# jwh97nn/AnyRef

Hardware: AMD Instinct MI355X
Metric: images/sec (1024^2, 7B LLM+ViT-L+SAM-H) (higher is better)
Workload: dtype bf16 (LLaMA / CLIP) + f16 (SAM encoder)

## Files before the change

### anyref_amd/_lib.py

```python
from __future__ import annotations

import ctypes as C
import os

import torch

HERE = os.path.dirname(os.path.abspath(__file__))
LIB_PATH = os.path.join(HERE, "libanyref_hip.so")

ABI_VERSION = 2
F32, BF16, F16 = 0, 1, 2
MODE_PARITY, MODE_PERF, MODE_PERF_FP8W, MODE_PARITY16 = 0, 1, 2, 3


class AnyrefConfig(C.Structure):
    _fields_ = [
        ("abi_version", C.c_int32), ("mode", C.c_int32),
        ("clip_image", C.c_int32), ("clip_patch", C.c_int32), ("clip_dim", C.c_int32),
        ("clip_heads", C.c_int32), ("clip_layers_run", C.c_int32), ("clip_mlp", C.c_int32),
        ("clip_eps", C.c_float),
        ("llm_vocab", C.c_int32), ("llm_dim", C.c_int32), ("llm_heads", C.c_int32),
        ("llm_layers", C.c_int32), ("llm_mlp", C.c_int32), ("llm_max_seq", C.c_int32),
        ("llm_rms_eps", C.c_float), ("llm_rope_theta", C.c_float),
        ("sam_img", C.c_int32), ("sam_patch", C.c_int32), ("sam_dim", C.c_int32), ("sam_depth", C.c_int32),
        ("sam_heads", C.c_int32), ("sam_mlp_ratio", C.c_int32), ("sam_window", C.c_int32),
        ("sam_n_global", C.c_int32), ("sam_global_idx", C.c_int32 * 8),
        ("sam_out_chans", C.c_int32), ("dec_heads", C.c_int32), ("dec_mlp", C.c_int32),
        ("dec_depth", C.c_int32), ("num_mask_tokens", C.c_int32),
        ("out_dim", C.c_int32), ("audio_dim", C.c_int32),
        ("seg_lo", C.c_int32), ("seg_hi", C.c_int32),
        ("rephrase_weight", C.c_float),
        ("max_batch", C.c_int32), ("max_seg", C.c_int32),
        ("aud_dim", C.c_int32), ("aud_blocks", C.c_int32), ("aud_heads", C.c_int32), ("aud_mel", C.c_int32),
        ("aud_len", C.c_int32), ("aud_kernel", C.c_int32), ("aud_stride", C.c_int32), ("aud_clips", C.c_int32),
    ]


_P = C.c_void_p
_I = C.c_int
_F = C.c_float
_L = C.c_int64

SYMBOLS = {
    "anyref_create": (_I, [C.POINTER(AnyrefConfig), _I, C.POINTER(_P)]),
    "anyref_destroy": (None, [_P]),
    "anyref_last_error": (C.c_char_p, [_P]),
    "anyref_set_weight": (_I, [_P, C.c_char_p, _P, _I, _I, C.POINTER(_L), _I]),
    "anyref_finalize": (_I, [_P]),
    "anyref_generate": (_I, [_P, _P, _P, _P, _P, _P, _I, _I, _P, _P, _I, _P, _P, _I, _I, _P, _P, _P, _P, _L, _P,
                             _P, _P]),
    "anyref_forward_teacher": (_I, [_P, _P, _P, _P, _P, _P, _I, _I, _P, _P, _I, _P, _P, _P, _P, _P, _L, _P, _P,
                                    _P, _P]),
    "anyref_encode_images": (_I, [_P, _P, _P, _I, _P, _P]),
    "anyref_sam_encode": (_I, [_P, _P, _P, _I, _P]),
    "anyref_mask_decode": (_I, [_P, _P, _P, _P, _I, _P, _P, _P, _P, _P]),
    "anyref_llm_forward": (_I, [_P, _P, _P, _P, _I, _I, _P, _P, _P, _P]),
    "anyref_project_audio": (_I, [_P, _P, _P, _I, _P]),
    "anyref_audio_encode": (_I, [_P, _P, _P, _I, _P]),
    "anyref_seg_tail": (_I, [_P, _P, _P, _P, _P, _P, _I, _I, _I, _P, _I, _P, _P, _P, _P, _P, _L, _P, _P]),
    "anyref_set_seg_range": (_I, [_P, _I, _I]),
    "anyref_set_overlap": (_I, [_P, _I]),
    "anyref_set_early_tail": (_I, [_P, _I]),
    "anyref_set_extra_event": (_I, [_P, _P]),
    "anyref_set_graphs": (_I, [_P, _I]),
    "anyref_set_side_share": (_I, [_P, _I, _I]),
    "anyref_profile_enable": (_I, [_P, _I]),
    "anyref_profile_config": (_I, [_P, C.c_char_p, _I]),
    "anyref_profile_collect": (_I, [_P]),
    "anyref_profile_calibrate": (_I, [_P, _P, C.POINTER(C.c_double)]),
    "anyref_profile_read": (_I, [_P, _I, C.c_char_p, _I, C.POINTER(C.c_double), C.POINTER(_L),
                                C.POINTER(C.c_double), C.POINTER(C.c_double)]),
    "anyref_stamps_enable": (_I, [_P, _I]),
    "anyref_stamps_collect": (_I, [_P, C.POINTER(_L)]),
    "anyref_stamps_dropped": (_I, [_P, C.POINTER(_L)]),
    "anyref_stamps_read": (_I, [_P, _L, C.c_char_p, _I, C.POINTER(C.c_double), C.POINTER(C.c_double),
                               C.POINTER(C.c_double), C.POINTER(_I)]),
    "anyref_stamps_spread": (_I, [_P, _L, C.POINTER(C.c_double), C.POINTER(C.c_double), C.POINTER(C.c_double)]),
    "anyref_device_bytes": (_L, [_P]),
    "anyref_mode_name": (C.c_char_p, [_P]),
    "anyref_op_gemm": (_I, [_I, _P, _P, _P, _P, _P, _P, _P, _I, _I, _I, _I, _I]),
    "anyref_op_gemm_fp8": (_I, [_P, _P, _P, _P, _P, _P, _P, _I, _I, _I, _I, _I]),
    "anyref_op_quant_fp8": (_I, [_P, _P, _I, _I, _P, _P]),
    "anyref_op_gemv_fp8": (_I, [_P, _P, _P, _F, _P, _P, _P, _P, _P, _P, _I, _I, _I]),
    "anyref_op_iou_counts": (_I, [_P, _P, _P, _I, _L, _P]),
    "anyref_op_avs_counts": (_I, [_P, _P, _P, _I, _L, _P, _I, _F, _P, _P]),
    "anyref_op_sam_preprocess": (_I, [_P, _P, _I, _I, _I, C.POINTER(C.c_float), C.POINTER(C.c_float), _P]),
    "anyref_op_pil_resample_u8": (_I, [_P, _P, _I, _I, _I, _P, _P, _I, _I, _P, _P, _I, _P, _P, _I]),
    "anyref_op_pool_ref_tokens": (_I, [_P, _P, _I, _I, _I, _I, _P]),
    "anyref_op_kaldi_fbank": (_I, [_P, _P, _I, _I, _I, _I, _I, C.c_float, _P, _I, _P, _P, _I, C.c_float, C.c_float, _P]),
    "anyref_op_clip_finish": (_I, [_P, _P, _I, _I, _I, _I, _I, _I, _I, C.POINTER(C.c_float), C.POINTER(C.c_float), _P]),
    "anyref_op_gemv": (_I, [_I, _P, _P, _P, _F, _P, _P, _P, _P, _P, _I, _I, _I, _I]),
    "anyref_op_norm": (_I, [_I, _P, _P, _P, _P, _P, _I, _I, _F, _I]),
    "anyref_op_attention": (_I, [_I, _P, _P, _P, _P, _P, _I, _I, _I, _I, _I, _F, _I, _P, _P, _P, _I, _I]),
    "anyref_op_attention_tab": (_I, [_I, _P, _P, _P, _P, _P, _I, _I, _I, _I, _F, _P, _P, _I, _I, _I]),
    "anyref_op_gemm_gather": (_I, [_I, _P, _P, _P, _P, _P, _P, _P, _I, _I, _I, _I]),
    "anyref_op_attention_relp": (_I, [_I, _P, _P, _P, _P, _P, _I, _I, _I, _I, _F, _P, _I, _I, _I]),
    "anyref_op_rel_pos": (_I, [_I, _P, _P, _P, _P, _I, _I, _I, _I, _P, _P]),
    "anyref_op_postprocess": (_I, [_P, _P, _I, _I, _I, _I, _I, _I, _I, _I, _P]),
    "anyref_op_last_error": (C.c_char_p, []),
}

_lib = None


def load() -> C.CDLL:
    global _lib
    if _lib is not None:
        return _lib
    if not os.path.exists(LIB_PATH):
        raise RuntimeError(
            f"{LIB_PATH} not found: build the HIP backend first "
            "(`python -c 'import __graft_entry__ as g; g.build()'` or `make -C anyref_amd/csrc`). "
            "anyref_amd has no CPU fallback.")
    lib = C.CDLL(LIB_PATH)
    for name, (res, args) in SYMBOLS.items():
        fn = getattr(lib, name)
        fn.restype = res
        fn.argtypes = args
    _lib = lib
    return lib
```

### anyref_amd/csrc/gemm_impl.h

```cpp
#include <algorithm>
#include <cmath>
#include <cstdlib>
#include <stdexcept>
#include <type_traits>
#include <utility>
#include <vector>
#include <mutex>

#pragma once
#include "kernels.h"

namespace anyref {

template <typename T>
struct Mma;
template <>
struct Mma<bf16> {
  static constexpr int KS = 32;
  static constexpr int VEC = 8;
  using Frag = short8;
  static __device__ inline Frag load(const bf16* p, int lane) {
    return *reinterpret_cast<const short8*>(p + 8 * (lane >> 4));
  }
  static __device__ inline float4v mma(Frag a, Frag b, float4v c) {
// ... 280 lines not shown
                  ? *reinterpret_cast<const uint4v*>(A + (int64_t)gm * a.lda + gk)
                  : uint4v{0, 0, 0, 0};
    }
#pragma unroll
    for (int i = 0; i < WV; ++i) {
      const int v = tid + i * 256, row = v / KV, kv = v % KV;
      const int gn = n0 + row, gk = k0 + kv * VEC;
      rw[i] = (gn < a.N && gk < a.K)
                  ? *reinterpret_cast<const uint4v*>(W + (int64_t)gn * a.ldw + gk)
                  : uint4v{0, 0, 0, 0};
    }
  };
  auto sstore = [&]() {
#pragma unroll
    for (int i = 0; i < AV; ++i) {
      const int v = tid + i * 256, row = v / KV, kv = v % KV;
      *reinterpret_cast<uint4v*>(&As[row * LD + kv * VEC]) = ra[i];
    }
#pragma unroll
    for (int i = 0; i < WV; ++i) {
      const int v = tid + i * 256, row = v / KV, kv = v % KV;
      *reinterpret_cast<uint4v*>(&Ws[row * LD + kv * VEC]) = rw[i];
    }
  };

  gload(0);
  for (int k0 = 0; k0 < a.K; k0 += BK) {
    sstore();
    __syncthreads();
    if (k0 + BK < a.K) gload(k0 + BK);
#pragma unroll
    for (int ks = 0; ks < BK / KS; ++ks) {
      typename M_::Frag af[MI], bf[NI];
#pragma unroll
      for (int i = 0; i < MI; ++i)
        af[i] = M_::load(&As[(wr * (BM / 2) + i * 16 + (lane & 15)) * LD + ks * KS], lane);
#pragma unroll
      for (int j = 0; j < NI; ++j)
        bf[j] = M_::load(&Ws[(wc * (BN / 2) + j * 16 + (lane & 15)) * LD + ks * KS], lane);
#pragma unroll
      for (int i = 0; i < MI; ++i)
#pragma unroll
        for (int j = 0; j < NI; ++j) acc[i][j] = M_::mma(bf[j], af[i], acc[i][j]);
    }
    __syncthreads();
  }

  gemm_epilogue<T, MI, NI>(a, acc, m0 + wr * (BM / 2), n0 + wc * (BN / 2), z, lane);
}

typedef const __attribute__((address_space(1))) void* gas_ptr;
typedef __attribute__((address_space(3))) void* las_ptr;

template <int N>
__device__ __forceinline__ void wait_vmcnt() {
  asm volatile("s_waitcnt vmcnt(%0)" ::"n"(N) : "memory");
}

__device__ __forceinline__ short8 fp8x8_to_bf16x8(uint2v r) {
  short8 o;
#pragma unroll
  for (int h = 0; h < 2; ++h) {
    const float2v lo = __builtin_amdgcn_cvt_pk_f32_fp8((int)r[h], false);
    const float2v hi = __builtin_amdgcn_cvt_pk_f32_fp8((int)r[h], true);
    o[4 * h] = (short)f2bf(lo[0]).x; o[4 * h + 1] = (short)f2bf(lo[1]).x;
    o[4 * h + 2] = (short)f2bf(hi[0]).x; o[4 * h + 3] = (short)f2bf(hi[1]).x;
  }
  return o;
}

template <int BM, int BN, int WM, int WN, int NS, bool W8 = false, bool PERSIST = false, typename TT = bf16>
__global__ __launch_bounds__(WM * WN * 64) void gemm_glds_kernel(GemmArgs a) {
  using T = TT;
  constexpr bool SPLIT = is_split<TT>::value;
  using ET = std::conditional_t<SPLIT, bf16, TT>;
  constexpr int AX = SPLIT ? 2 : 1;
  static_assert(!W8 || !(is_half16<T>::value || SPLIT), "fp8 weights are widened to bf16");
  constexpr int BK = 64, NW = WM * WN;
  constexpr int TM = BM / WM, TN = BN / WN, MI = TM / 16, NI = TN / 16;
  constexpr int ROWB = BK * 2;
  constexpr int WROWB = W8 ? BK : BK * 2;
  constexpr int WRPI = W8 ? 16 : 8;
  constexpr int TILEB = BM * ROWB + BN * WROWB;
  constexpr int RA = BM / (NW * 8), RWF = BN / (NW * WRPI), PW = (BN % (NW * WRPI)) / WRPI, RW = RWF + (PW > 0);
  constexpr int LPT = RA + RWF;
#ifdef ANYREF_GEMM_NO_PAIRW
  constexpr bool PAIRW = false;
#else
  constexpr bool PAIRW = !W8 && !(NI % 2 == 1 && BM < 256);
#endif
  constexpr int NIP = PAIRW ? (NI & ~1) : 0;
  static_assert(BM % (NW * 8) == 0 && BN % WRPI == 0 && (PW == 0 || !W8), "tile rows must split over the waves");
  static_assert(NS >= 2 && NS <= 4 && (NS - 2) * (LPT + 1) <= 63, "stage count / vmcnt range");
  extern __shared__ __attribute__((aligned(1024))) char smem[];
  const int tid = threadIdx.x, lane = tid & 63, wave = __builtin_amdgcn_readfirstlane(tid >> 6);
  const int wr = wave / WN, wc = wave % WN;
  auto wswz = [](int row) { return PAIRW ? ((row >> 1) & 1) | (((row >> 3) & 3) << 1) : (row >> 1) & 7; };
  auto wrow = [&](int f) {
    const int i = lane & 15;
    return wc * TN + (f < NIP ? (f >> 1) * 32 + 8 * (i >> 2) + 4 * (f & 1) + (i & 3) : f * 16 + i);
  };
  const int tiles_m = cdiv(a.M, BM), tiles_n = cdiv(a.N, BN), nwg = tiles_m * tiles_n;
  for (int vb = blockIdx.x; vb < nwg; vb += gridDim.x) {
  int id = vb;
  if (a.order & 1) {
    const int q = nwg / 8, r = nwg % 8, xcd = id % 8;
    id = (xcd < r ? xcd * (q + 1) : r * (q + 1) + (xcd - r) * q) + id / 8;
  }
  int tm, tn;
  if (a.group_m > 0) {
    const int per = a.group_m * tiles_n, g = id / per, first = g * a.group_m;
    const int gsz = tiles_m - first < a.group_m ? tiles_m - first : a.group_m;
    tm = first + (id % per) % gsz;
    tn = (id % per) / gsz;
  } else {
    tm = (a.order & 2) ? id % tiles_m : id / tiles_n;
    tn = (a.order & 2) ? id / tiles_m : id % tiles_n;
  }
  const int m0 = tm * BM, n0 = tn * BN;
  const int z = blockIdx.z;
  const ET* __restrict__ A = reinterpret_cast<const ET*>(a.A) + (int64_t)z * a.sA * AX;
  using WT = std::conditional_t<W8, uint8_t, ET>;
  const WT* __restrict__ W = reinterpret_cast<const WT*>(a.W) + (int64_t)z * a.sW;

  float4v acc[MI][NI];
#pragma unroll
  for (int i = 0; i < MI; ++i)
#pragma unroll
    for (int j = 0; j < NI; ++j) acc[i][j] = float4v{0.f, 0.f, 0.f, 0.f};

  const int srow = lane >> 3, sp = lane & 7;
  const ET* asrc[RA];
  const WT* wsrc[RW];
#pragma unroll
  for (int r = 0; r < RA; ++r) {
    const int row = (r * NW + wave) * 8 + srow;
    int gm = m0 + row;
    gm = gm < a.M ? gm : a.M - 1;
    if (a.a_row_map) gm = a.a_row_map[gm];
    asrc[r] = A + (int64_t)gm * a.lda * AX + ((sp ^ ((row >> 1) & 7)) << 3);
  }
#pragma unroll
  for (int r = 0; r < RW; ++r) {
    if constexpr (W8) {
      const int row = (r * NW + wave) * 16 + (lane >> 2);
      int gn = n0 + row;
      gn = gn < a.N ? gn : a.N - 1;
      wsrc[r] = W + (int64_t)gn * a.ldw + (((lane & 3) ^ ((row >> 2) & 3)) << 4);
    } else {
      const int row = (r * NW + wave) * 8 + srow;
      int gn = n0 + row;
      gn = gn < a.N ? gn : a.N - 1;
      wsrc[r] = W + (int64_t)gn * a.ldw + ((sp ^ wswz(row)) << 3);
    }
  }
  auto stage = [&](auto buf_c, int t) {
    constexpr int buf = decltype(buf_c)::value;
    char* base = smem + buf * TILEB;
#pragma unroll
    for (int r = 0; r < RA; ++r)
      __builtin_amdgcn_global_load_lds((gas_ptr)(asrc[r] + t * BK), (las_ptr)(base + (r * NW + wave) * 8 * ROWB), 16, 0,
                                       0);
#pragma unroll
    for (int r = 0; r < RW; ++r)
      if (r < RWF || wave < PW)
        __builtin_amdgcn_global_load_lds((gas_ptr)(wsrc[r] + (SPLIT ? t >> 1 : t) * BK),
                                         (las_ptr)(base + BM * ROWB + (r * NW + wave) * WRPI * WROWB), 16, 0, 0);
  };
  auto wait_tiles = [&](auto n_c) {
    constexpr int N = decltype(n_c)::value;
    if constexpr (PW == 0 || N == 0) {
      wait_vmcnt<N * LPT>();
    } else {
      if (wave < PW) wait_vmcnt<N * (LPT + 1)>();
      else wait_vmcnt<N * LPT>();
    }
  };
  constexpr bool QUAD = BM == 256 && WM == 2 && !W8 && MI == 8 && NI == 4;
  auto compute_quad = [&](auto buf_c) {
    constexpr int buf = decltype(buf_c)::value;
    constexpr int MH = MI / 2, NH0 = NI / 2, NH1 = NI - NH0;
    const char* Ab = smem + buf * TILEB;
    const char* Wb = Ab + BM * ROWB;
    short8 a0[2][MH], a1[2][MH], b0[2][NH0], b1[2][NH1];
    auto lda = [&](auto i_c, short8 (&af)[2][MH]) {
#pragma unroll
      for (int ks = 0; ks < 2; ++ks)
#pragma unroll
        for (int f = 0; f < MH; ++f) {
          const int row = wr * TM + (decltype(i_c)::value * MH + f) * 16 + (lane & 15), c = ks * 4 + (lane >> 4);
          af[ks][f] = *reinterpret_cast<const short8*>(Ab + row * ROWB + ((c ^ ((row >> 1) & 7)) << 4));
        }
    };
    auto ldw0 = [&]() {
#pragma unroll
      for (int ks = 0; ks < 2; ++ks)
#pragma unroll
        for (int f = 0; f < NH0; ++f) {
          const int row = wrow(f), c = ks * 4 + (lane >> 4);
          b0[ks][f] = *reinterpret_cast<const short8*>(Wb + row * ROWB + ((c ^ wswz(row)) << 4));
        }
    };
    auto ldw1 = [&]() {
#pragma unroll
      for (int ks = 0; ks < 2; ++ks)
#pragma unroll
        for (int f = 0; f < NH1; ++f) {
          const int row = wrow(NH0 + f), c = ks * 4 + (lane >> 4);
          b1[ks][f] = *reinterpret_cast<const short8*>(Wb + row * ROWB + ((c ^ wswz(row)) << 4));
        }
    };
    auto mma = [&](auto i_c, auto j_c, const short8 (&af)[2][MH], const auto& bf) {
      constexpr int i = decltype(i_c)::value, j = decltype(j_c)::value, NH = j == 0 ? NH0 : NH1;
      __builtin_amdgcn_s_setprio(1);
#pragma unroll
      for (int ks = 0; ks < 2; ++ks)
#pragma unroll
        for (int f = 0; f < MH; ++f)
#pragma unroll
          for (int h = 0; h < NH; ++h)
            acc[i * MH + f][j * NH0 + h] =
                mfma_16x16x32<ET>(bf[ks][h], af[ks][f], acc[i * MH + f][j * NH0 + h]);
      __builtin_amdgcn_s_setprio(0);
    };
    using I0 = std::integral_constant<int, 0>;
    using I1 = std::integral_constant<int, 1>;
    ldw0();
    lda(I0(), a0);
    ldw1();
    mma(I0(), I0(), a0, b0);
    lda(I1(), a1);
    mma(I0(), I1(), a0, b1);
    mma(I1(), I1(), a1, b1);
    mma(I1(), I0(), a1, b0);
  };
  auto compute = [&](auto buf_c) {
    if constexpr (QUAD) {
      compute_quad(buf_c);
      return;
    }
    constexpr int buf = decltype(buf_c)::value;
    const char* Ab = smem + buf * TILEB;
    const char* Wb = Ab + BM * ROWB;
#pragma unroll
    for (int ks = 0; ks < BK / 32; ++ks) {
      short8 af[MI], bfr[NI];
      const int c = ks * 4 + (lane >> 4);
#pragma unroll
      for (int i = 0; i < MI; ++i) {
        const int row = wr * TM + i * 16 + (lane & 15);
        af[i] = *reinterpret_cast<const short8*>(Ab + row * ROWB + ((c ^ ((row >> 1) & 7)) << 4));
      }
#pragma unroll
      for (int j = 0; j < NI; ++j) {
        const int row = wrow(j);
        if constexpr (W8) {
          const int g = lane >> 4, c8 = ks * 2 + (g >> 1);
// ... 86 lines not shown
      float4v acc;
      if constexpr (SP > 0) {
        float4v t[SP];
#pragma unroll
        for (int z = 0; z < SP; ++z) t[z] = *reinterpret_cast<const float4v*>(slabs + z * slab_stride + e);
        acc = t[0];
#pragma unroll
        for (int z = 1; z < SP; ++z) acc += t[z];
      } else {
        acc = *reinterpret_cast<const float4v*>(slabs + e);
        for (int z = 1; z < splits; ++z) acc += *reinterpret_cast<const float4v*>(slabs + z * slab_stride + e);
      }
      acc *= a.alpha;
      if (a.col_scale) acc *= *reinterpret_cast<const float4v*>(a.col_scale + n);
      if (a.bias) acc += *reinterpret_cast<const float4v*>(a.bias + n);
      acc = float4v{apply_act(acc[0], a.act), apply_act(acc[1], a.act), apply_act(acc[2], a.act), apply_act(acc[3], a.act)};
      if (a.resid) acc += *reinterpret_cast<const float4v*>(a.resid + (int64_t)m * a.ldr + n);
      if (a.c_f32) {
        *reinterpret_cast<float4v*>(Cf + (int64_t)m * a.ldc + n) = acc;
      } else if constexpr (is_split<T>::value) {
        st4<T>(Ct + (int64_t)m * a.ldc, n, acc[0], acc[1], acc[2], acc[3]);
      } else {
        T* o = Ct + (int64_t)m * a.ldc + n;
        o[0] = from_f32<T>(acc[0]); o[1] = from_f32<T>(acc[1]); o[2] = from_f32<T>(acc[2]); o[3] = from_f32<T>(acc[3]);
      }
      v[i] = acc;
      ss += acc[0] * acc[0] + acc[1] * acc[1] + acc[2] * acc[2] + acc[3] * acc[3];
    } else {
      v[i] = float4v{0.f, 0.f, 0.f, 0.f};
    }
  }
  __shared__ float red[NT / 64];
  float mean = 0.f;
  if (a.norm_bias) {
    float s1 = 0.f;
#pragma unroll
    for (int i = 0; i < MAXV; ++i) s1 += v[i][0] + v[i][1] + v[i][2] + v[i][3];
    s1 = wave_sum(s1);
    if ((tid & 63) == 0) red[tid >> 6] = s1;
    __syncthreads();
    float tot1 = 0.f;
#pragma unroll
    for (int w = 0; w < NT / 64; ++w) tot1 += red[w];
    mean = tot1 / (float)a.N;
    __syncthreads();
    ss = 0.f;
#pragma unroll
    for (int i = 0; i < MAXV; ++i) {
      if (tid + i * NT < nv) {
        v[i] -= mean;
        ss += v[i][0] * v[i][0] + v[i][1] * v[i][1] + v[i][2] * v[i][2] + v[i][3] * v[i][3];
      }
    }
  }
  ss = wave_sum(ss);
  if ((tid & 63) == 0) red[tid >> 6] = ss;
  __syncthreads();
  float tot = 0.f;
#pragma unroll
  for (int w = 0; w < NT / 64; ++w) tot += red[w];
  const float scale = rsqrtf(tot / (float)a.N + a.norm_eps);
  T* y = reinterpret_cast<T*>(a.norm_out) + (int64_t)m * a.norm_ld;
#pragma unroll
  for (int i = 0; i < MAXV; ++i) {
    const int c = tid + i * NT;
    if (c < nv) {
      const int n = c * 4;
      const float4v g = *reinterpret_cast<const float4v*>(a.norm_gain + n);
      float4v o = v[i] * scale * g;
      if (a.norm_bias) o += *reinterpret_cast<const float4v*>(a.norm_bias + n);
      st4<T>(y, n, o[0], o[1], o[2], o[3]);
    }
  }
}

float* splitk_workspace(hipStream_t s, size_t bytes);

struct GemmKnobs {
  bool no_glds = getenv("ANYREF_GEMM_NO_GLDS") != nullptr;
  bool no_splitk = getenv("ANYREF_GEMM_NO_SPLITK") != nullptr;
  int gm = getenv("ANYREF_GEMM_GM") ? atoi(getenv("ANYREF_GEMM_GM")) : -1;
  int tile = getenv("ANYREF_GEMM_TILE") ? atoi(getenv("ANYREF_GEMM_TILE")) : -1;
  int m320 = getenv("ANYREF_GEMM_M320") ? atoi(getenv("ANYREF_GEMM_M320")) : 0;
  int ns320 = getenv("ANYREF_GEMM_NS320") ? atoi(getenv("ANYREF_GEMM_NS320")) : 3;
  int force128 = getenv("ANYREF_GEMM_FORCE128") ? atoi(getenv("ANYREF_GEMM_FORCE128")) : 0;
};
static const GemmKnobs& knobs() {
  static const GemmKnobs k;
  return k;
}

template <typename T>
void launch_gemm(const GemmArgs& a_in, hipStream_t s) {
  GemmArgs a = a_in;
  if (a.norm_done) *a.norm_done = false;
  if (a.swiglu_pairs && (a.N % 4 || a.bias || a.resid || a.row_map || a.act != ACT_NONE || a.batch != 1))
    throw std::runtime_error("gemm: the SwiGLU epilogue takes interleaved gate/up rows, N % 4 == 0, and nothing else");
  constexpr int VEC = Mma<T>::VEC;
  constexpr bool SP = is_split<T>::value;
  constexpr bool IS16 = sizeof(T) == 2 || SP;
  if constexpr (SP) {
    if (a.K % 64 || a.lda % 64 || a.sA % 64 || a.w_fp8 || (!a.c_f32 && !a.slabs_out && (a.ldc % 64 || a.sC % 64)) ||
        (a.norm_out && a.norm_ld % 64))
      throw std::runtime_error("gemm<sp16>: K, lda, the A batch stride (and ldc of a split-pair output) must be multiples of 64");
  }
  if (a.slabs_out && a.slabs > 1) {
    if (!IS16 || a.batch != 1 || a.row_map || a.bias || a.resid || a.act != ACT_NONE || a.swiglu_pairs || a.w_fp8 ||
        a.K % (64 * a.slabs))
      throw std::runtime_error("gemm: raw split-K slabs take a plain bf16 product with K % (64 * slabs) == 0");
    GemmArgs g = a;
    g.K = a.K / a.slabs;
    g.batch = a.slabs;
    g.sA = g.K;
    g.sW = g.K;
    g.C = a.slabs_out; g.ldc = a.N; g.sC = (int64_t)a.M * a.N; g.c_f32 = 1;
    g.slabs_out = nullptr; g.slabs = 0; g.norm_out = nullptr;
    launch_gemm<T>(g, s);
    return;
  }
  if (!knobs().no_splitk && IS16 && a.batch == 1 && !a.row_map && a.M <= 512 &&
      (a.K >= 2048 || (a.K >= 1024 && a.norm_out && a.norm_bias)) && a.N % 4 == 0 && a.ldc % 4 == 0 &&
      (!a.resid || a.ldr % 4 == 0)) {
    const int64_t tiles = (int64_t)cdiv(a.M, 128) * cdiv(a.N, 128);
    int splits = 1;
    while (splits < 8 && tiles * splits < 256 && (a.K / (splits * 2)) % 64 == 0 && a.K / (splits * 2) >= 512) splits *= 2;
    if (splits > 1) {
      const int64_t slab = (int64_t)a.M * a.N;
      float* ws = splitk_workspace(s, (size_t)splits * slab * sizeof(float));
      GemmArgs g = a;
      g.K = a.K / splits;
      g.batch = splits;
      g.sA = g.K;
      g.sW = g.K;
      g.C = ws; g.ldc = a.N; g.sC = slab; g.c_f32 = 1;
      g.bias = nullptr; g.resid = nullptr; g.act = ACT_NONE; g.alpha = 1.f; g.col_scale = nullptr; g.swiglu_pairs = 0;
      launch_gemm<T>(g, s);
      if (a.norm_out && a.norm_gain && a.N <= 8192 && a.norm_ld % 4 == 0 && !a.swiglu_pairs) {
        auto rn = [&](auto nt_t, auto sp_t, auto mv_t) {
          constexpr int NT = decltype(nt_t)::value, SP = decltype(sp_t)::value, MV = decltype(mv_t)::value;
          hipLaunchKernelGGL((splitk_reduce_norm_kernel<T, NT, SP, MV>), dim3(a.M), dim3(NT), 0, s, ws, splits, slab, a);
        };
        using C0 = std::integral_constant<int, 0>;
        using C1 = std::integral_constant<int, 1>;
        using C2 = std::integral_constant<int, 2>;
        using C4 = std::integral_constant<int, 4>;
        using C8 = std::integral_constant<int, 8>;
        using C256 = std::integral_constant<int, 256>;
        using C1024 = std::integral_constant<int, 1024>;
        if (a.N <= 1024) {
          if (splits == 8) rn(C256(), C8(), C1());
          else if (splits == 2) rn(C256(), C2(), C1());
          else rn(C256(), C0(), C1());
        } else if (a.N <= 4096) {
          if (splits == 4) rn(C1024(), C4(), C1());
          else rn(C1024(), C0(), C1());
        } else {
          if (splits == 4) rn(C1024(), C4(), C2());
          else rn(C1024(), C0(), C2());
        }
        if (a.norm_done) *a.norm_done = true;
        return;
      }
      const int64_t total = slab / 4;
      const int grid = (int)(cdiv64(total, 256) < 2048 ? cdiv64(total, 256) : 2048);
      hipLaunchKernelGGL((splitk_reduce_kernel<T>), dim3(grid), dim3(256), 0, s, ws, splits, slab, a);
      return;
    }
  }
  constexpr int BK = sizeof(T) == 2 ? 64 : 16;
  if (a.M <= 0 || a.N <= 0) return;
  if (a.a_row_map && (!IS16 || a.K % 64 || knobs().no_glds || knobs().tile >= 0 || a.batch != 1))
    throw std::runtime_error("gemm: a_row_map is taken by the 16-bit LDS-DMA kernel only (K % 64 == 0, batch 1)");
  if (a.K % VEC || a.lda % VEC || a.ldw % VEC || ((uintptr_t)a.A & 15) || ((uintptr_t)a.W & 15) ||
      (a.sA % VEC) || (a.sW % VEC))
    throw std::runtime_error("gemm: K/lda/ldw must be multiples of 16 bytes and operands 16-byte aligned");
  const int64_t t128 = (int64_t)cdiv(a.M, 128) * cdiv(a.N, 128) * a.batch;
  const int64_t t64x128 = (int64_t)cdiv(a.M, 64) * cdiv(a.N, 128) * a.batch;
  bool bm128;
  int bn;
  if (a.M <= 512) {
    bm128 = false;
    bn = t64x128 >= 384 ? 128 : 64;
  } else if (t128 >= 512) {
    bm128 = true;
    bn = 128;
  } else {
    bm128 = false;
    bn = t64x128 >= 256 ? 128 : 64;
  }
  if (knobs().tile >= 0) {
    const int v = knobs().tile;
    bm128 = v & 2;
    bn = (v & 1) ? 128 : 64;
  }
  dim3 block(256);
  a.order = 3;
  {
    const int ov = a.c_f32 ? 4 : (int)sizeof(T);
    const bool al = a.N % 4 == 0 && a.ldc % 4 == 0 && a.sC % 4 == 0 && !((uintptr_t)a.C & 15) &&
                    (!a.resid || (a.ldr % 4 == 0 && a.sR % 4 == 0 && !((uintptr_t)a.resid & 15))) &&
                    (!a.bias || (a.sBias % 4 == 0 && !((uintptr_t)a.bias & 15)));
    a.vec_ok = al && (ov == 4 || ov == 2) ? 1 : 0;
    if (a.swiglu_pairs) a.vec_ok = (a.N % 4 == 0 && a.ldc % 2 == 0 && !((uintptr_t)a.C & 3) && (!a.col_scale || !((uintptr_t)a.col_scale & 15))) ? 1 : 0;
  }
  const double flops = 2.0 * a.M * a.N * (double)a.K * a.batch;
  const double wbytes = a.w_fp8 ? 1.0 : (SP ? 2.0 : (double)sizeof(T));
  const double bytes = ((double)a.M * a.K * sizeof(T) + (double)a.N * a.K * wbytes) * a.batch +
                       (double)a.M * a.N * (a.c_f32 ? 4 : sizeof(T)) * a.batch;
  if (a.w_fp8 && (sizeof(T) != 2 || a.K % 64 || knobs().no_glds || knobs().tile >= 0))
    throw std::runtime_error("gemm: an fp8 weight operand needs the bf16 LDS-DMA kernel (K % 64 == 0)");
  if constexpr (IS16) {
    if (SP || (!knobs().no_glds && a.K % 64 == 0 && knobs().tile < 0)) {
      auto go = [&](auto bm_t, auto bn_t, auto wm_t, auto wn_t, auto ns_t, const char* tag) {
        constexpr int BM = decltype(bm_t)::value, BN = decltype(bn_t)::value, WM = decltype(wm_t)::value,
                      WN = decltype(wn_t)::value, NS = decltype(ns_t)::value;
        constexpr size_t lds = NS * (size_t)(BM + BN) * 128;
        if constexpr (BN % (WM * WN * 16) == 0 && !is_half16<T>::value && !SP) {
          if (a.w_fp8) {
            auto kern8 = &gemm_glds_kernel<BM, BN, WM, WN, NS, true>;
            static KernelAttrOnce once8;
            ensure_dyn_lds(once8, reinterpret_cast<const void*>(kern8), (int)lds);
            const int tiles_m8 = cdiv(a.M, BM), nwg8 = tiles_m8 * cdiv(a.N, BN);
            int gm8 = (int)lround(sqrt((double)(nwg8 > 8 ? nwg8 / 8 : 1)));
            a.group_m = gm8 < 1 ? 1 : (gm8 > tiles_m8 ? tiles_m8 : gm8);
            char tag8[56];
            snprintf(tag8, sizeof(tag8), "%s_fp8w%s", tag, a.M <= 16 ? "_dec" : "");
            ProfScope prof(tag8, flops, bytes, s);
            hipLaunchKernelGGL(kern8, dim3(nwg8, 1, a.batch), dim3(WM * WN * 64), NS * ((size_t)BM * 128 + (size_t)BN * 64),
                               s, a);
            return;
          }
        }
        auto kern = &gemm_glds_kernel<BM, BN, WM, WN, NS, false, false, T>;
        static KernelAttrOnce once;
        ensure_dyn_lds(once, reinterpret_cast<const void*>(kern), (int)lds);
        {
          const int tiles_m = cdiv(a.M, BM), nwg = tiles_m * cdiv(a.N, BN);
          int gm = (int)lround(sqrt((double)(nwg > 8 ? nwg / 8 : 1)));
          gm = gm < 1 ? 1 : (gm > tiles_m ? tiles_m : gm);
          a.group_m = knobs().gm >= 0 ? knobs().gm : gm;
        }
        char tagt[56];
        snprintf(tagt, sizeof(tagt), "%s%s%s", SP ? "gemm_sp16_" : is_half16<T>::value ? "gemm_f16_" : "gemm_bf16_", tag + 10,
                 a.M <= 16 ? "_dec" : "");
        ProfScope prof(tagt, flops, bytes, s);
        dim3 grid(cdiv(a.N, BN) * cdiv(a.M, BM), 1, a.batch);
        if constexpr (BM <= 256 && BM >= 128) {
          const int cap = a.max_wg / 8 * 8 * (lds * 2 <= 160 * 1024 ? 2 : 1);
          if (cap >= 8 && a.batch == 1 && (int)grid.x > cap) {
            if constexpr (BM == 256) {
              const int tn = cdiv(a.N, BN), rows = std::max(1, cap / tn) * BM;
              for (int m0 = 0; m0 < a.M; m0 += rows) {
                GemmArgs c = a;
                c.M = std::min(rows, a.M - m0);
                if (a.a_row_map) c.a_row_map = a.a_row_map + m0;
                else c.A = reinterpret_cast<const T*>(a.A) + (int64_t)m0 * a.lda;
                if (a.row_map) {
                  c.row_map = a.row_map + m0;
                } else {
                  c.C = a.c_f32 ? (void*)(reinterpret_cast<float*>(a.C) + (int64_t)m0 * a.ldc)
                                : (void*)(reinterpret_cast<T*>(a.C) + (int64_t)m0 * a.ldc);
                  if (a.resid) c.resid = a.resid + (int64_t)m0 * a.ldr;
                }
                const int tiles_m = cdiv(c.M, BM), nwg = tiles_m * tn;
                int gm = (int)lround(sqrt((double)(nwg > 8 ? nwg / 8 : 1)));
                c.group_m = gm < 1 ? 1 : (gm > tiles_m ? tiles_m : gm);
                hipLaunchKernelGGL(kern, dim3(nwg, 1, 1), dim3(WM * WN * 64), lds, s, c);
              }
              return;
            } else {
              auto kp = &gemm_glds_kernel<BM, BN, WM, WN, NS, false, true, T>;
              static KernelAttrOnce oncep;
              ensure_dyn_lds(oncep, reinterpret_cast<const void*>(kp), (int)lds);
              hipLaunchKernelGGL(kp, dim3(cap), dim3(WM * WN * 64), lds, s, a);
              return;
            }
          }
        }
        hipLaunchKernelGGL(kern, grid, dim3(WM * WN * 64), lds, s, a);
      };
      using I1 = std::integral_constant<int, 1>;
      using I2 = std::integral_constant<int, 2>;
      using I3 = std::integral_constant<int, 3>;
      using I4 = std::integral_constant<int, 4>;
      using I64 = std::integral_constant<int, 64>;
      using I128 = std::integral_constant<int, 128>;
      using I256 = std::integral_constant<int, 256>;
      const int cus = device_cus();
      const int64_t t256 = (int64_t)cdiv(a.M, 256) * cdiv(a.N, 256) * a.batch;
      const double fill256 = (double)t256 / (double)(cdiv64(t256, cus) * cus);
      const int64_t t64w = (int64_t)cdiv(a.M, 64) * cdiv(a.N, 256) * a.batch;
      const int64_t t128 = (int64_t)cdiv(a.M, 128) * cdiv(a.N, 128) * a.batch;
      using I320 = std::integral_constant<int, 320>;
      using I160 = std::integral_constant<int, 160>;
      const int64_t t160 = (int64_t)cdiv(a.M, 128) * cdiv(a.N, 160) * a.batch;
      const double fill160 = (double)t160 / (double)(cdiv64(t160, cus) * cus);
      const double fill128 = (double)t128 / (double)(cdiv64(t128, cus) * cus);
      const int64_t t320 = (int64_t)cdiv(a.M, 256) * cdiv(a.N, 320) * a.batch;
      const double fill320 = (double)t320 / (double)(cdiv64(t320, cus) * cus);
      if (a.M >= 1024 && knobs().force128 == 3) {
        go(I128(), I128(), I2(), I4(), I3(), "gemm_bf16_128x128s3");
        return;
      }
      if (a.M >= 1024 && knobs().force128 == 2) {
        go(I128(), I128(), I2(), I4(), I2(), "gemm_bf16_128x128g");
        return;
      }
      static const double fill256_min = getenv("ANYREF_GEMM_FILL256") ? atof(getenv("ANYREF_GEMM_FILL256")) : 0.80;
      if (a.M >= 1024 && fill256 >= fill256_min) {
        go(I256(), I256(), I2(), I4(), I2(), "gemm_bf16_256x256");
        return;
      }
      if (!a.w_fp8 && a.M >= 1024 && a.N % 320 == 0 && fill320 >= 0.95) {
        go(I256(), I320(), I2(), I4(), I2(), "gemm_bf16_256x320");
        return;
      }
      if (!a.w_fp8 && a.M >= 1024 && a.N % 160 == 0 && fill160 >= 0.95 && fill128 < 0.7) {
        go(I128(), I160(), I4(), I2(), I3(), "gemm_bf16_128x160s3");
        return;
      }
      if constexpr (!is_half16<T>::value) {
        if (!a.w_fp8 && knobs().m320 >= 0 && a.M > 192 && a.M <= 320 && a.N >= 16384 && a.batch == 1 && cdiv(a.N, 96) <= cus) {
          if (knobs().ns320 == 2) go(I320(), std::integral_constant<int, 96>(), I4(), I2(), I2(), "gemm_bf16_320x96");
          else go(I320(), std::integral_constant<int, 96>(), I4(), I2(), I3(), "gemm_bf16_320x96s3");
          return;
        }
        if (!a.w_fp8 && knobs().m320 >= 0 && a.M > 192 && a.M <= 320 && a.batch == 2 && a.N >= 8192 &&
            (int64_t)cdiv(a.N, 96) * 2 <= cus) {
          if (knobs().ns320 == 2) go(I320(), std::integral_constant<int, 96>(), I4(), I2(), I2(), "gemm_bf16_320x96");
          else go(I320(), std::integral_constant<int, 96>(), I4(), I2(), I3(), "gemm_bf16_320x96s3");
          return;
        }
        if (!a.w_fp8 && knobs().m320 >= 0 && a.M > 192 && a.M <= 320 && a.batch > 1 && (int64_t)cdiv(a.N, 64) * a.batch <= cus &&
            (int64_t)cdiv(a.N, 64) * a.batch * 4 >= cus * 3) {
          go(I320(), I64(), I4(), I2(), I3(), "gemm_bf16_320x64");
          return;
        }
        {
          static const bool m320x4 = !(getenv("ANYREF_GEMM_M320X4") && atoi(getenv("ANYREF_GEMM_M320X4")) == 0);
          const int64_t t320x64 = (int64_t)cdiv(a.M, 320) * cdiv(a.N, 64);
          if (m320x4 && !a.w_fp8 && a.batch == 1 && a.M > 512 && a.M <= 2560 && a.K >= 2048 && t320x64 <= cus && t320x64 * 10 >= cus * 9 &&
              fill128 < 0.7) {
            go(I320(), I64(), I4(), I2(), I3(), "gemm_bf16_320x64");
            return;
          }
        }
        if (a.M <= 512 && a.N >= 8192) {
          if (t64w <= cus) go(I64(), I256(), I1(), I4(), I3(), "gemm_bf16_64x256s3");
          else go(I64(), I256(), I1(), I4(), I2(), "gemm_bf16_64x256");
          return;
        }
      }
      if constexpr (!is_half16<T>::value) {
        static const bool clip64 = !(getenv("ANYREF_GEMM_CLIP64") && atoi(getenv("ANYREF_GEMM_CLIP64")) == 0);
        if (clip64 && !a.w_fp8 && a.batch == 1 && a.M > 128 && a.M <= 320 && a.N >= 2048 && a.N < 8192 && a.K <= 2048 && t128 <= cus) {
          go(I64(), I128(), I1(), I4(), I3(), "gemm_bf16_64x128s3");
          return;
        }
      }
      if (t128 <= cus)
        go(I128(), I128(), I2(), I4(), I3(), "gemm_bf16_128x128s3");
      else
        go(I128(), I128(), I2(), I4(), I2(), "gemm_bf16_128x128g");
      return;
    }
  }
  if constexpr (SP) {
    throw std::runtime_error("gemm<sp16>: no register-staged fallback (unreachable)");
  } else {
  const char* tag = is_half16<T>::value ? (bm128 ? (bn == 128 ? "gemm_f16_128x128" : "gemm_f16_128x64")
                                                 : (bn == 128 ? "gemm_f16_64x128" : "gemm_f16_64x64"))
                    : sizeof(T) == 2 ? (bm128 ? (bn == 128 ? "gemm_bf16_128x128" : "gemm_bf16_128x64")
                                            : (bn == 128 ? "gemm_bf16_64x128" : "gemm_bf16_64x64"))
                                   : (bm128 ? (bn == 128 ? "gemm_f32_128x128" : "gemm_f32_128x64")
                                            : (bn == 128 ? "gemm_f32_64x128" : "gemm_f32_64x64"));
  ProfScope prof(tag, flops, bytes, s);
  if (bm128 && bn == 128) {
    dim3 grid(cdiv(a.N, 128) * cdiv(a.M, 128), 1, a.batch);
    hipLaunchKernelGGL((gemm_kernel<T, 128, 128, BK>), grid, block, 0, s, a);
  } else if (bm128) {
    dim3 grid(cdiv(a.N, 64) * cdiv(a.M, 128), 1, a.batch);
    hipLaunchKernelGGL((gemm_kernel<T, 128, 64, BK>), grid, block, 0, s, a);
  } else if (bn == 128) {
    dim3 grid(cdiv(a.N, 128) * cdiv(a.M, 64), 1, a.batch);
    hipLaunchKernelGGL((gemm_kernel<T, 64, 128, BK>), grid, block, 0, s, a);
  } else {
    dim3 grid(cdiv(a.N, 64) * cdiv(a.M, 64), 1, a.batch);
    hipLaunchKernelGGL((gemm_kernel<T, 64, 64, BK>), grid, block, 0, s, a);
  }
  }
}

}
```

### anyref_amd/csrc/optest.hip

```cpp
#include <algorithm>
#include <string>
#include <vector>

#include "../../include/anyref_hip_ops.h"
#include "kernels.h"

using namespace anyref;

static thread_local std::string g_op_err;

#define OP_GUARD(body)                                   \
  try {                                                  \
    body;                                                \
    hipError_t _e = hipGetLastError();                   \
    if (_e != hipSuccess) {                              \
      g_op_err = std::string("HIP error: ") + hipGetErrorString(_e); \
      return 3;                                          \
    }                                                    \
    return 0;                                            \
  } catch (const std::exception& e) {                    \
    g_op_err = e.what();                                 \
    return 2;                                            \
  }

// ... 100 lines not shown

int anyref_op_attention_tab(int t, void* stream, const void* q, const void* k, const void* v, void* o, int B, int H, int S,
                            int hd, float scale, const void* tab_h, const void* tab_w, int tab_ld, int kh, int kw) {
  OP_GUARD({
    AttnArgs a;
    a.Q = q; a.K = k; a.V = v; a.O = o;
    a.q_bs = a.k_bs = a.v_bs = a.o_bs = (int64_t)S * H * hd;
    a.q_rs = a.k_rs = a.v_rs = a.o_rs = H * hd; a.q_hs = a.k_hs = a.v_hs = a.o_hs = hd;
    a.B = B; a.H = H; a.Sq = S; a.Sk = S; a.hd = hd; a.scale = scale;
    a.rel_tab_h = tab_h; a.rel_tab_w = tab_w; a.rel_tab_ld = tab_ld; a.kh = kh; a.kw = kw;
    if (t == 3) {
      if ((H * hd) % 64) throw std::runtime_error("op_attention_tab t=3: H * hd % 64 != 0");
      if (!attention_takes_rel_tables(4, hd, S, S, kh, kw, true)) throw std::runtime_error("op_attention_tab t=3: not a window shape");
      TmpBuf Os((size_t)B * S * H * hd * 4);
      a.O = Os.p; a.o_split = 1; a.sp16 = 1;
      launch_attention<float>(a, (hipStream_t)stream);
      launch_unsplit(Os.p, H * hd, reinterpret_cast<float*>(o), H * hd, B * S, H * hd, (hipStream_t)stream);
    } else
    if (t == 2) launch_attention<f16>(a, (hipStream_t)stream);
    else launch_attention<bf16>(a, (hipStream_t)stream);
  });
}

int anyref_op_gemm_gather(int t, void* stream, const void* A, const int32_t* a_row_map, const void* W, const float* bias,
                          void* C, const float* resid, int M, int N, int K, int c_f32) {
  OP_GUARD({
    GemmArgs a;
    a.A = A; a.lda = K; a.W = W; a.ldw = K; a.bias = bias; a.C = C; a.ldc = N; a.resid = resid; a.ldr = N;
    a.a_row_map = a_row_map; a.M = M; a.N = N; a.K = K; a.c_f32 = c_f32;
    if (t == 2) launch_gemm<f16>(a, (hipStream_t)stream);
    else if (t == 1) launch_gemm<bf16>(a, (hipStream_t)stream);
    else throw std::runtime_error("gemm_gather: 16-bit types only");
  });
}

int anyref_op_attention_relp(int t, void* stream, const void* q, const void* k, const void* v, void* o, int B, int H, int S,
                             int hd, float scale, const float* rel_p, int rel_ld, int kh, int kw) {
  OP_GUARD({
    AttnArgs a;
    a.Q = q; a.K = k; a.V = v; a.O = o;
    a.q_bs = a.k_bs = a.v_bs = a.o_bs = (int64_t)S * H * hd;
    a.q_rs = a.k_rs = a.v_rs = a.o_rs = H * hd; a.q_hs = a.k_hs = a.v_hs = a.o_hs = hd;
    a.B = B; a.H = H; a.Sq = S; a.Sk = S; a.hd = hd; a.scale = scale;
    a.rel_p = rel_p; a.rel_ld = rel_ld; a.rel_hs = (int64_t)B * S * rel_ld; a.kh = kh; a.kw = kw;
    if (t == 3) {
      if ((H * hd) % 64) throw std::runtime_error("op_attention_relp t=3: H * hd % 64 != 0");
      TmpBuf Os((size_t)B * S * H * hd * 4);
      a.O = Os.p; a.o_split = 1; a.sp16 = 1;
      launch_attention<float>(a, (hipStream_t)stream);
      launch_unsplit(Os.p, H * hd, reinterpret_cast<float*>(o), H * hd, B * S, H * hd, (hipStream_t)stream);
    } else
    if (t == 0) launch_attention<float>(a, (hipStream_t)stream);
    else if (t == 2) launch_attention<f16>(a, (hipStream_t)stream);
    else launch_attention<bf16>(a, (hipStream_t)stream);
  });
}

int anyref_op_rel_pos(int t, void* stream, const void* q, const float* tab_h, const float* tab_w, int B, int H,
                      int size, int hd, float* rel_h, float* rel_w) {
  OP_GUARD({
    const int64_t S = (int64_t)size * size;
    if (t == 0)
      launch_rel_pos<float>(q, S * H * hd, H * hd, hd, tab_h, tab_w, B, H, size, hd, rel_h, rel_w, (hipStream_t)stream);
    else
      launch_rel_pos<bf16>(q, S * H * hd, H * hd, hd, tab_h, tab_w, B, H, size, hd, rel_h, rel_w, (hipStream_t)stream);
  });
}

int anyref_op_postprocess(void* stream, const float* low, int n, int lh, int lw, int S, int rh, int rw, int H, int W,
                          float* out) {
  OP_GUARD(launch_postprocess(low, (int64_t)lh * lw, n, lh, lw, S, rh, rw, H, W, out, (hipStream_t)stream));
}

int anyref_op_gemm_fp8(void* stream, const void* A, const uint8_t* W8, const float* scale, const float* bias, void* C,
                       const float* resid, int M, int N, int K, int act, int c_f32) {
  OP_GUARD({
    GemmArgs a;
    a.A = A; a.lda = K; a.W = W8; a.ldw = K; a.w_fp8 = 1; a.col_scale = scale; a.bias = bias; a.C = C; a.ldc = N;
    a.resid = resid; a.ldr = N; a.M = M; a.N = N; a.K = K; a.act = act; a.c_f32 = c_f32;
    launch_gemm<bf16>(a, (hipStream_t)stream);
  });
}

int anyref_op_quant_fp8(void* stream, const float* src, int N, int K, uint8_t* q, float* scale) {
  OP_GUARD(launch_quant_fp8_rows(src, K, N, K, q, K, scale, (hipStream_t)stream));
}

int anyref_op_gemv_fp8(void* stream, const float* x, const float* gain, float eps, const uint8_t* W,
                       const uint8_t* W2, const float* scale, const float* scale2, float* y, const float* resid,
                       int B, int N, int K) {
  OP_GUARD({
    GemvArgs a;
    a.x = x; a.ldx = K; a.gain = gain; a.eps = eps; a.W = W; a.W2 = W2; a.wscale = scale; a.wscale2 = scale2;
    a.w_fp8 = 1; a.y = y; a.resid = resid; a.ldy = N; a.B = B; a.N = N; a.K = K;
    launch_gemv<bf16>(a, (hipStream_t)stream);
  });
}

int anyref_op_iou_counts(void* stream, const float* logits, const uint8_t* target, int n, int64_t hw,
                         int64_t* counts) {
  OP_GUARD(launch_iou_counts(logits, target, n, hw, counts, (hipStream_t)stream));
}

int anyref_op_avs_counts(void* stream, const float* logits, const uint8_t* target, int n, int64_t hw,
                         const float* cuts, int nth, float cut_pred, int64_t* conf, int64_t* hist) {
  OP_GUARD(launch_avs_counts(logits, target, n, hw, cuts, nth, cut_pred, conf, hist, (hipStream_t)stream));
}

int anyref_op_sam_preprocess(void* stream, const uint8_t* img, int h, int w, int S, const float* mean3,
                             const float* std3, float* out) {
  OP_GUARD(launch_sam_preprocess(img, h, w, S, mean3, std3, out, (hipStream_t)stream));
}

int anyref_op_pil_resample_u8(void* stream, const uint8_t* in, int H, int W, int C, uint8_t* tmp, uint8_t* out, int ow,
                              int oh, const int32_t* xbounds, const int32_t* xk, int kx, const int32_t* ybounds,
                              const int32_t* yk, int ky) {
  OP_GUARD(launch_pil_resample_u8(in, H, W, C, tmp, out, ow, oh, xbounds, xk, kx, ybounds, yk, ky, (hipStream_t)stream));
}

int anyref_op_pool_ref_tokens(void* stream, const float* feats, int n, int L, int H, int n_out, float* out) {
  OP_GUARD(launch_pool_ref_tokens(feats, n, L, H, n_out, out, (hipStream_t)stream));
}

int anyref_op_kaldi_fbank(void* stream, const float* wave, int C, int T, int win, int shift, int padded, float preemph,
                          const float* banks, int n_mel, const double* tw, double* scratch, int target_len, float mean,
                          float stdv, float* out) {
  OP_GUARD(launch_kaldi_fbank(wave, C, T, win, shift, padded, preemph, banks, n_mel, tw, scratch, target_len, mean, stdv, out,
                              (hipStream_t)stream));
}
int anyref_op_clip_finish(void* stream, const uint8_t* img, int ih, int iw, int y0, int x0, int h, int w, int S,
                          const float* mean3, const float* std3, float* out) {
  OP_GUARD(launch_clip_finish(img, ih, iw, y0, x0, h, w, S, mean3, std3, out, (hipStream_t)stream));
}
}
```

### include/anyref_hip_ops.h

```cpp
#ifndef ANYREF_HIP_OPS_H
#define ANYREF_HIP_OPS_H
#include <stdint.h>
#ifdef __cplusplus
extern "C" {
#endif

int anyref_op_gemm(int t, void* stream, const void* A, const void* W, const float* bias, void* C,
                   const float* resid, const int32_t* row_map, int M, int N, int K, int act, int c_f32);
int anyref_op_gemv(int t, void* stream, const float* x, const float* gain, float eps, const void* W,
                   const void* W2, const float* bias, float* y, const float* resid, int B, int N, int K, int act);
int anyref_op_norm(int t, void* stream, const float* x, const float* gain, const float* bias, float* y, int M,
                   int D, float eps, int rms);
int anyref_op_attention(int t, void* stream, const void* q, const void* k, const void* v, void* o, int B, int H,
                        int Sq, int Sk, int hd, float scale, int causal, const int32_t* kv_len,
                        const float* rel_h, const float* rel_w, int kh, int kw);
int anyref_op_rel_pos(int t, void* stream, const void* q, const float* tab_h, const float* tab_w, int B, int H,
                      int size, int hd, float* rel_h, float* rel_w);
int anyref_op_quant_fp8(void* stream, const float* src, int N, int K, uint8_t* q, float* scale);
int anyref_op_gemm_fp8(void* stream, const void* A, const uint8_t* W8, const float* scale, const float* bias, void* C,
                       const float* resid, int M, int N, int K, int act, int c_f32);
int anyref_op_gemv_fp8(void* stream, const float* x, const float* gain, float eps, const uint8_t* W,
                       const uint8_t* W2, const float* scale, const float* scale2, float* y, const float* resid,
                       int B, int N, int K);
int anyref_op_iou_counts(void* stream, const float* logits, const uint8_t* target, int n, int64_t hw,
                         int64_t* counts);
int anyref_op_avs_counts(void* stream, const float* logits, const uint8_t* target, int n, int64_t hw,
                         const float* cuts, int nth, float cut_pred, int64_t* conf, int64_t* hist);
int anyref_op_sam_preprocess(void* stream, const uint8_t* img, int h, int w, int S, const float* mean3,
                             const float* std3, float* out);
int anyref_op_pil_resample_u8(void* stream, const uint8_t* in, int H, int W, int C, uint8_t* tmp, uint8_t* out,
                              int ow, int oh, const int32_t* xbounds, const int32_t* xk, int kx,
                              const int32_t* ybounds, const int32_t* yk, int ky);
int anyref_op_pool_ref_tokens(void* stream, const float* feats, int n, int L, int H, int n_out, float* out);
int anyref_op_clip_finish(void* stream, const uint8_t* img, int ih, int iw, int y0, int x0, int h, int w, int S,
                          const float* mean3, const float* std3, float* out);
int anyref_op_kaldi_fbank(void* stream, const float* wave, int C, int T, int win, int shift, int padded, float preemph,
                          const float* banks, int n_mel, const double* tw, double* scratch, int target_len, float mean,
                          float stdv, float* out);
int anyref_op_attention_tab(int t, void* stream, const void* q, const void* k, const void* v, void* o, int B, int H, int S,
                            int hd, float scale, const void* tab_h, const void* tab_w, int tab_ld, int kh, int kw);
int anyref_op_gemm_gather(int t, void* stream, const void* A, const int32_t* a_row_map, const void* W, const float* bias,
                          void* C, const float* resid, int M, int N, int K, int c_f32);
int anyref_op_attention_relp(int t, void* stream, const void* q, const void* k, const void* v, void* o, int B, int H, int S,
                             int hd, float scale, const float* rel_p, int rel_ld, int kh, int kw);
int anyref_op_postprocess(void* stream, const float* low, int n, int lh, int lw, int S, int rh, int rw, int H,
                          int W, float* out);
const char* anyref_op_last_error(void);

#ifdef __cplusplus
}
#endif
#endif
```

Baseline: 25.41.

## Route mid-size bf16 GEMMs to 160-row tiles with paired-tile XCD scheduling

Adds support for tile heights that do not split evenly across waves, with partial A-row loads and a matching vmcnt wait. With this, bf16 GEMMs of M in (192,320] are routed to new 160x192 and 160x128 tiles instead of 320x96/320x64. When there are two M tiles grouped together, the grid is padded to a multiple of 16 so tile pairs sharing weights land on the same XCD. A slab-GEMM test entry point is also exposed. The change trades larger register and LDS pressure, plus idle padded workgroups, for better weight reuse and CU coverage.

```diff
diff --git a/anyref_amd/_lib.py b/anyref_amd/_lib.py
--- a/anyref_amd/_lib.py
+++ b/anyref_amd/_lib.py
@@ -80,6 +80,7 @@
     "anyref_mode_name": (C.c_char_p, [_P]),
     "anyref_op_gemm": (_I, [_I, _P, _P, _P, _P, _P, _P, _P, _I, _I, _I, _I, _I]),
     "anyref_op_gemm_fp8": (_I, [_P, _P, _P, _P, _P, _P, _P, _I, _I, _I, _I, _I]),
+    "anyref_op_gemm_slabs": (_I, [_P, _P, _P, _P, _I, _I, _I, _I]),
     "anyref_op_quant_fp8": (_I, [_P, _P, _I, _I, _P, _P]),
     "anyref_op_gemv_fp8": (_I, [_P, _P, _P, _F, _P, _P, _P, _P, _P, _P, _I, _I, _I]),
     "anyref_op_iou_counts": (_I, [_P, _P, _P, _I, _L, _P]),
diff --git a/anyref_amd/csrc/gemm_impl.h b/anyref_amd/csrc/gemm_impl.h
--- a/anyref_amd/csrc/gemm_impl.h
+++ b/anyref_amd/csrc/gemm_impl.h
@@ -386,16 +386,17 @@
   constexpr int WROWB = W8 ? BK : BK * 2;
   constexpr int WRPI = W8 ? 16 : 8;
   constexpr int TILEB = BM * ROWB + BN * WROWB;
-  constexpr int RA = BM / (NW * 8), RWF = BN / (NW * WRPI), PW = (BN % (NW * WRPI)) / WRPI, RW = RWF + (PW > 0);
-  constexpr int LPT = RA + RWF;
+  constexpr int RAF = BM / (NW * 8), PA = (BM % (NW * 8)) / 8, RA = RAF + (PA > 0);
+  constexpr int RWF = BN / (NW * WRPI), PW = (BN % (NW * WRPI)) / WRPI, RW = RWF + (PW > 0);
+  constexpr int LPT = RAF + RWF;
 #ifdef ANYREF_GEMM_NO_PAIRW
   constexpr bool PAIRW = false;
 #else
-  constexpr bool PAIRW = !W8 && !(NI % 2 == 1 && BM < 256);
+  constexpr bool PAIRW = !W8 && !(NI % 2 == 1 && BM == 128);
 #endif
   constexpr int NIP = PAIRW ? (NI & ~1) : 0;
-  static_assert(BM % (NW * 8) == 0 && BN % WRPI == 0 && (PW == 0 || !W8), "tile rows must split over the waves");
-  static_assert(NS >= 2 && NS <= 4 && (NS - 2) * (LPT + 1) <= 63, "stage count / vmcnt range");
+  static_assert(BM % 8 == 0 && BN % WRPI == 0 && (PW == 0 || !W8), "tile rows must split over the waves");
+  static_assert(NS >= 2 && NS <= 4 && (NS - 2) * (LPT + (PA > 0) + (PW > 0)) <= 63, "stage count / vmcnt range");
   extern __shared__ __attribute__((aligned(1024))) char smem[];
   const int tid = threadIdx.x, lane = tid & 63, wave = __builtin_amdgcn_readfirstlane(tid >> 6);
   const int wr = wave / WN, wc = wave % WN;
@@ -405,12 +406,14 @@
     return wc * TN + (f < NIP ? (f >> 1) * 32 + 8 * (i >> 2) + 4 * (f & 1) + (i & 3) : f * 16 + i);
   };
   const int tiles_m = cdiv(a.M, BM), tiles_n = cdiv(a.N, BN), nwg = tiles_m * tiles_n;
-  for (int vb = blockIdx.x; vb < nwg; vb += gridDim.x) {
+  const int nid = (a.order & 4) ? (nwg + 15) / 16 * 16 : nwg;
+  for (int vb = blockIdx.x; vb < nid; vb += gridDim.x) {
   int id = vb;
   if (a.order & 1) {
-    const int q = nwg / 8, r = nwg % 8, xcd = id % 8;
+    const int q = nid / 8, r = nid % 8, xcd = id % 8;
     id = (xcd < r ? xcd * (q + 1) : r * (q + 1) + (xcd - r) * q) + id / 8;
   }
+  if (id >= nwg) continue;
   int tm, tn;
   if (a.group_m > 0) {
     const int per = a.group_m * tiles_n, g = id / per, first = g * a.group_m;
@@ -463,8 +466,9 @@
     char* base = smem + buf * TILEB;
 #pragma unroll
     for (int r = 0; r < RA; ++r)
-      __builtin_amdgcn_global_load_lds((gas_ptr)(asrc[r] + t * BK), (las_ptr)(base + (r * NW + wave) * 8 * ROWB), 16, 0,
-                                       0);
+      if (r < RAF || wave < PA)
+        __builtin_amdgcn_global_load_lds((gas_ptr)(asrc[r] + t * BK), (las_ptr)(base + (r * NW + wave) * 8 * ROWB), 16, 0,
+                                         0);
 #pragma unroll
     for (int r = 0; r < RW; ++r)
       if (r < RWF || wave < PW)
@@ -473,10 +477,17 @@
   };
   auto wait_tiles = [&](auto n_c) {
     constexpr int N = decltype(n_c)::value;
-    if constexpr (PW == 0 || N == 0) {
+    if constexpr ((PA == 0 && PW == 0) || N == 0) {
       wait_vmcnt<N * LPT>();
     } else {
-      if (wave < PW) wait_vmcnt<N * (LPT + 1)>();
+      const int extra = (PA > 0 && wave < PA) + (PW > 0 && wave < PW);
+      if constexpr (PA > 0 && PW > 0) {
+        if (extra == 2) {
+          wait_vmcnt<N * (LPT + 2)>();
+          return;
+        }
+      }
+      if (extra == 1) wait_vmcnt<N * (LPT + 1)>();
       else wait_vmcnt<N * LPT>();
     }
   };
@@ -729,6 +740,7 @@
   int gm = getenv("ANYREF_GEMM_GM") ? atoi(getenv("ANYREF_GEMM_GM")) : -1;
   int tile = getenv("ANYREF_GEMM_TILE") ? atoi(getenv("ANYREF_GEMM_TILE")) : -1;
   int m320 = getenv("ANYREF_GEMM_M320") ? atoi(getenv("ANYREF_GEMM_M320")) : 0;
+  int m160 = getenv("ANYREF_GEMM_M160") ? atoi(getenv("ANYREF_GEMM_M160")) : 1;
   int ns320 = getenv("ANYREF_GEMM_NS320") ? atoi(getenv("ANYREF_GEMM_NS320")) : 3;
   int force128 = getenv("ANYREF_GEMM_FORCE128") ? atoi(getenv("ANYREF_GEMM_FORCE128")) : 0;
 };
@@ -887,12 +899,15 @@
           gm = gm < 1 ? 1 : (gm > tiles_m ? tiles_m : gm);
           a.group_m = knobs().gm >= 0 ? knobs().gm : gm;
         }
+        const bool pairs = BM == 160 && cdiv(a.M, BM) == 2 && a.group_m == 2 && (a.order & 1);
+        if (pairs) a.order |= 4;
         char tagt[56];
         snprintf(tagt, sizeof(tagt), "%s%s%s", SP ? "gemm_sp16_" : is_half16<T>::value ? "gemm_f16_" : "gemm_bf16_", tag + 10,
                  a.M <= 16 ? "_dec" : "");
         ProfScope prof(tagt, flops, bytes, s);
         dim3 grid(cdiv(a.N, BN) * cdiv(a.M, BM), 1, a.batch);
-        if constexpr (BM <= 256 && BM >= 128) {
+        if (pairs) grid.x = (grid.x + 15) / 16 * 16;
+        if constexpr (BM <= 256 && BM >= 128 && BM != 160) {
           const int cap = a.max_wg / 8 * 8 * (lds * 2 <= 160 * 1024 ? 2 : 1);
           if (cap >= 8 && a.batch == 1 && (int)grid.x > cap) {
             if constexpr (BM == 256) {
@@ -967,20 +982,25 @@
         return;
       }
       if constexpr (!is_half16<T>::value) {
+        const bool m160 = std::is_same<T, bf16>::value && knobs().m160 != 0;
+        using I192 = std::integral_constant<int, 192>;
         if (!a.w_fp8 && knobs().m320 >= 0 && a.M > 192 && a.M <= 320 && a.N >= 16384 && a.batch == 1 && cdiv(a.N, 96) <= cus) {
-          if (knobs().ns320 == 2) go(I320(), std::integral_constant<int, 96>(), I4(), I2(), I2(), "gemm_bf16_320x96");
+          if (m160) go(I160(), I192(), I2(), I4(), I3(), "gemm_bf16_160x192");
+          else if (knobs().ns320 == 2) go(I320(), std::integral_constant<int, 96>(), I4(), I2(), I2(), "gemm_bf16_320x96");
           else go(I320(), std::integral_constant<int, 96>(), I4(), I2(), I3(), "gemm_bf16_320x96s3");
           return;
         }
         if (!a.w_fp8 && knobs().m320 >= 0 && a.M > 192 && a.M <= 320 && a.batch == 2 && a.N >= 8192 &&
             (int64_t)cdiv(a.N, 96) * 2 <= cus) {
-          if (knobs().ns320 == 2) go(I320(), std::integral_constant<int, 96>(), I4(), I2(), I2(), "gemm_bf16_320x96");
+          if (m160) go(I160(), I192(), I2(), I4(), I3(), "gemm_bf16_160x192");
+          else if (knobs().ns320 == 2) go(I320(), std::integral_constant<int, 96>(), I4(), I2(), I2(), "gemm_bf16_320x96");
           else go(I320(), std::integral_constant<int, 96>(), I4(), I2(), I3(), "gemm_bf16_320x96s3");
           return;
         }
         if (!a.w_fp8 && knobs().m320 >= 0 && a.M > 192 && a.M <= 320 && a.batch > 1 && (int64_t)cdiv(a.N, 64) * a.batch <= cus &&
             (int64_t)cdiv(a.N, 64) * a.batch * 4 >= cus * 3) {
-          go(I320(), I64(), I4(), I2(), I3(), "gemm_bf16_320x64");
+          if (m160) go(I160(), I128(), I2(), I4(), I3(), "gemm_bf16_160x128");
+          else go(I320(), I64(), I4(), I2(), I3(), "gemm_bf16_320x64");
           return;
         }
         {
diff --git a/anyref_amd/csrc/optest.hip b/anyref_amd/csrc/optest.hip
--- a/anyref_amd/csrc/optest.hip
+++ b/anyref_amd/csrc/optest.hip
@@ -206,6 +206,15 @@
   });
 }
 
+int anyref_op_gemm_slabs(void* stream, const void* A, const void* W, float* slabs_out, int M, int N, int K, int slabs) {
+  OP_GUARD({
+    GemmArgs a;
+    a.A = A; a.lda = K; a.W = W; a.ldw = K; a.M = M; a.N = N; a.K = K;
+    a.slabs_out = slabs_out; a.slabs = slabs;
+    launch_gemm<bf16>(a, (hipStream_t)stream);
+  });
+}
+
 int anyref_op_quant_fp8(void* stream, const float* src, int N, int K, uint8_t* q, float* scale) {
   OP_GUARD(launch_quant_fp8_rows(src, K, N, K, q, K, scale, (hipStream_t)stream));
 }
diff --git a/include/anyref_hip_ops.h b/include/anyref_hip_ops.h
--- a/include/anyref_hip_ops.h
+++ b/include/anyref_hip_ops.h
@@ -19,6 +19,7 @@
 int anyref_op_quant_fp8(void* stream, const float* src, int N, int K, uint8_t* q, float* scale);
 int anyref_op_gemm_fp8(void* stream, const void* A, const uint8_t* W8, const float* scale, const float* bias, void* C,
                        const float* resid, int M, int N, int K, int act, int c_f32);
+int anyref_op_gemm_slabs(void* stream, const void* A, const void* W, float* slabs_out, int M, int N, int K, int slabs);
 int anyref_op_gemv_fp8(void* stream, const float* x, const float* gain, float eps, const uint8_t* W,
                        const uint8_t* W2, const float* scale, const float* scale2, float* y, const float* resid,
                        int B, int N, int K);
```

Result: faster. 25.69 (median of 6 runs) (+1.1%).
